# chalharu/rust-compression

Hardware: AMD Instinct MI355X
Metric: BZip2 level-9 encode MB/s (input bytes, HBM-resident in and out: the kernels' rate; value_end_to_end is host buffer to host buffer at the C ABI) (higher is better)
Workload: dtype u8/u32

## Files before the change

rust-compression_amd/csrc/k_bwt.hip:

```cpp
#include "bzgpu.h"
#include <algorithm>
#include <atomic>
#include <cstdio>
#include <cstdlib>
#include <vector>

namespace bzgpu {
constexpr u32 kGhSpan = 8;
constexpr u32 kSymSpan = 8;

enum { SRC_TEXT = 0, SRC_PAIRS = 1, SRC_MM = 2, SRC_WALK = 3, SRC_SURV = 4, SRC_LISTG = 5,
       SRC_TEXTK = 6, SRC_WALKK = 7, SRC_MMK = 8,
       SRC_MMC = 9,
       SRC_PERJ = 10,
       SRC_PACKED = 11,
       SRC_PERJK = 12,
       SRC_WALKA = 13 };
template <int SRC> struct src_is_list {
    static constexpr bool value = (SRC == SRC_PAIRS || SRC == SRC_SURV || SRC == SRC_LISTG || SRC == SRC_PERJ || SRC == SRC_PERJK || SRC == SRC_PACKED);
};

struct KeyInfo {
    u8 bits;
    u8 chars;
// ... 582 lines not shown
#pragma unroll
    for (u32 k = 0; k < 16; ++k) {
        const u32 i = k * kSortThreads + threadIdx.x;
        if (i < total) Vout[base + dst[k]] = s_buf[i];
    }
}

template <int B0, int B1, int B2>
__global__ __launch_bounds__(kSortThreads) void k_ghist_text(BwtArgs a, u32 *__restrict__ Kstore)
{
    constexpr u32 NB0 = 1u << B0, NB1 = 1u << B1, NB2 = 1u << B2;
    __shared__ u32 s_h0[2][NB0], s_h1[2][NB1], s_h2[2][NB2];
    u32 tile, lb;
    xcd_remap(gridDim.x, a.nb, tile, lb);
    if (lb == 0xFFFFFFFFu) return;
    const BlockDesc d = a.blocks[lb];
    const u32 n = d.n;
    const u32 start0 = tile * kGhSpan * kSortTile;
    if (start0 >= n) return;
    const u8 *text = a.rle + d.rle_off;
    const u8 *pt = a.ptext + (size_t)lb * kPtSlot;
    const KeyInfo ki = reinterpret_cast<const KeyInfo *>(a.keyinfo)[lb];
    if (B0 == 10 && B1 == 10 && B2 == 10 && !Kstore && counts_from_pack(ki)) return;
    for (u32 i = threadIdx.x; i < 2 * NB0; i += kSortThreads) (&s_h0[0][0])[i] = 0;
    for (u32 i = threadIdx.x; i < 2 * NB1; i += kSortThreads) (&s_h1[0][0])[i] = 0;
    for (u32 i = threadIdx.x; i < 2 * NB2; i += kSortThreads) (&s_h2[0][0])[i] = 0;
    __syncthreads();
    const u32 w = threadIdx.x >> 6, l = threadIdx.x & 63u;
    const size_t base = (size_t)lb * kSlot;
#pragma unroll 1
    for (u32 sp = 0; sp < kGhSpan; ++sp) {
        const u32 start = start0 + sp * kSortTile;
        if (start >= n) break;
        u32 key[16], val[16];
        const u32 ok = fetch_rows<SRC_TEXT>(a, lb, pt, n, 0, nullptr, nullptr, start + w * 1024u + l, n, ki, key, val);
#pragma unroll
        for (u32 r = 0; r < 16; ++r) {
            if ((ok >> r) & 1u) {
                atomicAdd(&s_h0[l & 1u][key[r] & (NB0 - 1)], 1u);
                atomicAdd(&s_h1[l & 1u][(key[r] >> B0) & (NB1 - 1)], 1u);
                atomicAdd(&s_h2[l & 1u][(key[r] >> (B0 + B1)) & (NB2 - 1)], 1u);
                if (Kstore) Kstore[base + start + w * 1024u + r * 64u + l] = key[r];
            }
        }
    }
    __syncthreads();
    u32 *out = a.gh_tiles + ((size_t)lb * kTilesPerBlock + tile) * 3 * kMaxBins;
    for (u32 i = threadIdx.x; i < NB0; i += kSortThreads) out[i] = s_h0[0][i] + s_h0[1][i];
    for (u32 i = threadIdx.x; i < NB1; i += kSortThreads) out[kMaxBins + i] = s_h1[0][i] + s_h1[1][i];
    for (u32 i = threadIdx.x; i < NB2; i += kSortThreads) out[2 * kMaxBins + i] = s_h2[0][i] + s_h2[1][i];
}

__global__ __launch_bounds__(kSortThreads) void k_ghist_scan(BwtArgs a, u32 ndig, u32 nbins0, u32 nbins1, u32 nbins2,
                                                             u32 ntiles_from_count, u32 span = 1u, u32 pack_counts = 0u)
{
    __shared__ u32 s_wsum[kSortThreads / 64];
    const u32 lb = blockIdx.x;
    const u32 n = a.blocks[lb].n;
    const u32 len = ntiles_from_count ? a.count[lb] : n;
    const u32 ntiles = ((len + kSortTile - 1) / kSortTile + span - 1u) / span;
    const u32 *gt = a.gh_tiles + (size_t)lb * kTilesPerBlock * 3 * kMaxBins;
    u32 total0 = 0;
    const bool one_set = pack_counts && counts_from_pack(reinterpret_cast<const KeyInfo *>(a.keyinfo)[lb]);
    if (one_set) ndig = 1;
    for (u32 dpos = 0; dpos < ndig; ++dpos) {
        const u32 nbins = dpos == 0 ? nbins0 : (dpos == 1 ? nbins1 : nbins2);
        const u32 per = (nbins + kSortThreads - 1) / kSortThreads;
        u32 tot[4] = {0, 0, 0, 0};
        u32 mine = 0;
        for (u32 q = 0; q < per; ++q) {
            const u32 bin = threadIdx.x * per + q;
            u32 sum = 0;
            if (bin < nbins)
                for (u32 t = 0; t < ntiles; ++t) sum += gt[(size_t)t * 3 * kMaxBins + dpos * kMaxBins + bin];
            tot[q] = sum;
            mine += sum;
        }
        const u32 inc = wave_incl_sum(mine);
        __syncthreads();
        if ((threadIdx.x & 63u) == 63u) s_wsum[threadIdx.x >> 6] = inc;
        __syncthreads();
        u32 carry = 0, total = 0;
        for (u32 k = 0; k < kSortThreads / 64; ++k) {
            if (k < (threadIdx.x >> 6)) carry += s_wsum[k];
            total += s_wsum[k];
        }
        u32 run = carry + inc - mine;
        for (u32 q = 0; q < per; ++q) {
            const u32 bin = threadIdx.x * per + q;
            if (bin < nbins) {
                a.gbase[((size_t)lb * 3 + dpos) * kMaxBins + bin] = run;
                if (one_set) {
                    a.gbase[((size_t)lb * 3 + 1) * kMaxBins + bin] = run;
                    a.gbase[((size_t)lb * 3 + 2) * kMaxBins + bin] = run;
                }
            }
            run += tot[q];
        }
        if (dpos == 0) total0 = total;
    }
    if (threadIdx.x == 0) a.count[lb] = total0;
}

#ifdef BZ_SCATTER_TIMING
#define SC_T(k) do { __syncthreads(); const u64 t_ = __builtin_readcyclecounter(); if (threadIdx.x == 0) atomicAdd(&a.loc_stats[32 + ((SRC == SRC_PAIRS || SRC == SRC_PACKED) ? 0 : 8) + (k)], (u32)((t_ - t_prev) >> 6)); t_prev = t_; } while (0)
#else
#define SC_T(k) do { } while (0)
#endif
template <int SRC, int BITS, bool WRITE_K = true, bool PACK_OUT = false, int ROWS = 16, int TILE = (int)kSortTile>
__global__ __launch_bounds__(TILE / ROWS) void k_radix_scatter_lb(BwtArgs a, u32 shift, u32 h,
                                                                    const u32 *__restrict__ Kin,
                                                                    const u32 *__restrict__ Vin,
                                                                    u32 *__restrict__ Kout, u32 *__restrict__ Vout,
                                                                    u32 dpos, u32 epoch,
                                                                    const u32 *__restrict__ gate)
{
    constexpr u32 NB = 1u << BITS;
    constexpr u32 kT = (u32)TILE / ROWS;
    static_assert((u32)TILE == kSortTile, "the look-back words are laid out for tiles of kSortTile elements");
    constexpr u32 kTileStride = kTilesPerBlock;
    u32 *const tstate = a.tile_state;
    constexpr u32 kRows = ROWS;
// ... 744 lines not shown
        if (h_next < n) atomicAdd(&a.active[round], (unsigned long long)s_nonfinal);
    }
    {
        const u32 b0 = threadIdx.x * 2u;
        const u32 c0 = s_bcnt[b0], c1 = s_bcnt[b0 + 1];
        const u32 mine = c0 + c1;
        const u32 inc = wave_incl_sum(mine);
        if (l == 63) s_wsum[w] = inc;
        u32 g0 = 0, g1 = 0;
        u32 *cur = a.bin_cursor + (size_t)lb * 1024u;
        if (c0) g0 = atomicAdd(&cur[b0], c0);
        if (c1) g1 = atomicAdd(&cur[b0 + 1], c1);
        __syncthreads();
        u32 carry = 0;
        for (u32 k = 0; k < w; ++k) carry += s_wsum[k];
        const u32 ex = carry + inc - mine;
        s_bpre[b0] = (u16)ex;
        s_bpre[b0 + 1] = (u16)(ex + c0);
        s_bcnt[b0] = (b0 << kRankBinShift) + g0;
        s_bcnt[b0 + 1] = ((b0 + 1u) << kRankBinShift) + g1;
    }
    __syncthreads();
#pragma unroll
    for (u32 r = 0; r < 16; ++r) {
        if (lrank[r] != 0xFFFFFFFFu) {
            const u32 bin = jv[r] >> kRankBinShift;
            const u32 pos = (u32)s_bpre[bin] + lrank[r];
            s_stage[pos] = word[r];
            s_binof[pos] = (u16)bin;
        }
    }
    __syncthreads();
    const u32 total = (cnt - start) < kSortTile ? (cnt - start) : kSortTile;
#pragma unroll
    for (u32 k = 0; k < 16; ++k) {
        const u32 i = k * kSortThreads + threadIdx.x;
        if (i < total) {
            const u32 bin = s_binof[i];
            W[base + s_bcnt[bin] + (i - (u32)s_bpre[bin])] = s_stage[i];
        }
    }
}

constexpr u32 kLbNone = 0xFFFFFu;
#ifdef BZ_REFINE_TIMING
#define RF_T(k) do { __syncthreads(); const u64 t_ = __builtin_readcyclecounter(); if (threadIdx.x == 0) atomicAdd(&a.loc_stats[16 + (INIT ? 8 : 0) + (k)], (u32)((t_ - t_prev) >> 4)); t_prev = t_; } while (0)
#else
#define RF_T(k) do { } while (0)
#endif
template <bool INIT, bool ABITS = false>
__global__ __launch_bounds__(kSortThreads, 4) void k_group_refine(BwtArgs a, u32 step, u32 next_step, u32 round,
                                                                const u32 *__restrict__ K,
                                                                const u32 *__restrict__ V, u32 *__restrict__ W,
                                                                u32 epoch)
{
    constexpr u32 NW = kSortThreads / 64;
    __shared__ int s_carry_old, s_carry_new;
    __shared__ int s_wold[NW], s_wnew[NW];
    __shared__ u32 s_nonfinal, s_ticket;
    __shared__ u32 s_stage[kSortTile];
    __shared__ u16 s_binof[kSortTile];
    __shared__ u16 s_bpre[1024];
    __shared__ u16 s_bdst[1024];
    __shared__ u32 s_wsum[NW];
    u32 (*s_gh)[1024] = reinterpret_cast<u32 (*)[1024]>(s_stage);
    u32 *s_bcnt = s_stage + 2048;
#ifdef BZ_REFINE_TIMING
    u64 t_prev = __builtin_readcyclecounter();
#endif
    const u32 xcd = (u32)__builtin_amdgcn_s_getreg(20 | (3 << 11)) & 7u;
    const u32 my_tiles = a.tiles * ((a.nb + 7u - xcd) / 8u);
    if (threadIdx.x == 0) s_ticket = atomicAdd(&a.tickets[(size_t)epoch * 8u + xcd], 1u);
    __syncthreads();
    const u32 slot = s_ticket;
    if (slot >= my_tiles) return;
    const u32 b8 = slot / a.tiles;
    const u32 tile = slot - b8 * a.tiles;
    const u32 lb = b8 * 8u + xcd;
    const BlockDesc d = a.blocks[lb];
    const u32 n = d.n;
    const u8 *__restrict__ text = a.rle + d.rle_off;
    const u32 cnt = a.count[lb];
    const u32 start = tile * kSortTile;
    if (start >= cnt) return;
    const KeyInfo ki = reinterpret_cast<const KeyInfo *>(a.keyinfo)[lb];
    const u32 hm = INIT ? (u32)ki.chars % n : (((u32)ki.chars * 2u) << step) % n;
    const u8 *pt = a.ptext + (size_t)lb * kPtSlot;
    const size_t base = (size_t)lb * kSlot;
    static_assert(INIT || !ABITS, "the boundary bitmap belongs to the init");
    if (INIT && !ABITS && a.pb_gate[lb] == 0u) K = a.KA;
    for (u32 i = threadIdx.x; i < 3072u; i += kSortThreads) s_stage[i] = 0;
    if (threadIdx.x == 0) s_nonfinal = 0;
    const u32 w = threadIdx.x >> 6, l = threadIdx.x & 63u;
    const u32 wbase = start + w * 1024u;
    const u32 first = wbase + l;

    RF_T(0);
    u32 gk[16], jv[16], s1[16], s2[16];
    u32 pg0 = 0, ps10 = 0, ps20 = 0;
    u32 ng0 = 0, ns10 = 0, ns20 = 0;
    const bool need_prev = (l == 0) && (first > 0) && (first < cnt);
    const bool need_next = (l == 63) && (wbase + 1024u < cnt);
    const u64 aword = ABITS ? newbits_lane_word(a.abits, base, wbase, cnt, l, false) : 0ull;
    {
#pragma unroll
        for (u32 r = 0; r < 16; ++r) {
            const u32 idx = first + r * 64u;
            const u32 c = idx < cnt ? idx : cnt - 1u;
            const u32 kk = ABITS ? 0u : ld_stream(K + base + c);
            const u32 vv = ld_stream(V + base + c);
            if (INIT) {
                jv[r] = vv;
                const u32 t = vv + hm;
                s2[r] = t >= n ? t - n : t;
                gk[r] = 0u;
                s1[r] = kk;
            } else {
                jv[r] = vv & 0xFFFFFu;
                gk[r] = kk & 0xFFFFFu;
                s1[r] = (kk >> 20) | ((vv >> 20) << 12);
                s2[r] = 0u;
            }
        }
        u32 pj = 0, nj = 0;
        if (need_prev) {
            const u32 kk = ABITS ? 0u : K[base + wbase - 1], vv = V[base + wbase - 1];
            pg0 = INIT ? 0u : (kk & 0xFFFFFu);
            ps10 = INIT ? kk : ((kk >> 20) | ((vv >> 20) << 12));
            const u32 t = vv + hm;
            pj = t >= n ? t - n : t;
        }
        if (need_next) {
            const u32 kk = ABITS ? 0u : K[base + wbase + 1024u], vv = V[base + wbase + 1024u];
            ng0 = INIT ? 0u : (kk & 0xFFFFFu);
            ns10 = INIT ? kk : ((kk >> 20) | ((vv >> 20) << 12));
            const u32 t = vv + hm;
            nj = t >= n ? t - n : t;
        }
        if (INIT) {
            pkey_rows(pt, s2, ki, s2);
            if (need_prev) ps20 = pkey(pt, pj, ki);
            if (need_next) ns20 = pkey(pt, nj, ki);
        }
    }
// ... 84 lines not shown
            }
            const u32 fi = etag | kLbIncl;
            const u32 io = lo >= 0 ? (u32)lo : (u32)co, in = ln >= 0 ? (u32)ln : (u32)cn;
            st_sc1_x4(mystate, make_uint4(fi | (io & kLbValMask), fi | (in & kLbValMask), fi, fi));
        }
        a.tile_last_new[lb * kTilesPerBlock + tile] = ln >= 0 ? ln : cn;
        a.tile_last_old[lb * kTilesPerBlock + tile] = lo >= 0 ? lo : co;
        s_carry_old = co;
        s_carry_new = cn;
    }
    __syncthreads();
    RF_T(3);
    int carry_old = INIT ? 0 : s_carry_old, carry_new = s_carry_new;
    for (u32 k = 0; k < w; ++k) {
        if (!INIT) carry_old = s_wold[k] > carry_old ? s_wold[k] : carry_old;
        carry_new = s_wnew[k] > carry_new ? s_wnew[k] : carry_new;
    }
    const u64 le_mask = (l == 63) ? ~0ull : ((2ull << l) - 1ull);
    u32 my_nonfinal = 0;
    u32 word[16], lrank[16];
#pragma unroll
    for (u32 r = 0; r < 16; ++r) {
        const u32 rowbase = wbase + r * 64u;
        const u32 idx = rowbase + l;
        lrank[r] = 0xFFFFFFFFu;
        word[r] = 0;
        bool nf = false;
        u32 nf_head = 0;
        if (idx < cnt) {
            int rs = 0;
            if (!INIT) {
                const u64 o = mo[r] & le_mask;
                rs = o ? (int)(rowbase + 63u - __clzll(o)) : carry_old;
            }
            const u64 q = mn[r] & le_mask;
            const int ss = q ? (int)(rowbase + 63u - __clzll(q)) : carry_new;
            const bool fin = (finbits >> r) & 1u;
            const u32 g = gk[r];
            const u32 j = jv[r];
            const u32 p = g + (idx - (u32)rs);
            const u32 head = g + ((u32)ss - (u32)rs);
            if (!INIT) st_stream(a.SA + base + p, j);
            if (fin) {
                a.L[base + p] = INIT ? (u8)lcol[r] : text[j ? j - 1u : n - 1u];
                if (j == 0) a.orig_ptr[lb] = p;
            }
            word[r] = (j & kRankBinMask) | (head << kRankBinShift) | (fin ? kFinalBit : 0u);
            lrank[r] = atomicAdd(&s_bcnt[j >> kRankBinShift], 1u);
            nf = !fin;
            nf_head = head;
        }
        {
            const u64 mnf = __ballot(nf);
            if (mnf) {
                my_nonfinal += (u32)__popcll(mnf);
                if (nf && (l == 0 || ((mn[r] >> l) & 1ull))) {
                    const u64 rest = (l == 63) ? 0ull : (mn[r] >> (l + 1u));
                    u32 len = rest ? (u32)__ffsll((long long)rest) : 64u - l;
                    len = len < cnt - idx ? len : cnt - idx;
                    atomicAdd(&s_gh[0][nf_head & 1023u], len);
                }
                const u32 lead = (u32)__ffsll((long long)mnf) - 1u;
                const u32 hi = (nf_head >> 10) & 1023u;
                const u32 hi0 = wave_lane(hi, lead);
                const u64 same = __ballot(nf && hi == hi0);
                if (same == mnf) {
                    if (l == lead) atomicAdd(&s_gh[1][hi0], (u32)__popcll(mnf));
                } else if (nf) {
                    atomicAdd(&s_gh[1][hi], 1u);
                }
            }
        }
        if (!INIT && mo[r]) carry_old = (int)(rowbase + 63u - __clzll(mo[r]));
        if (mn[r]) carry_new = (int)(rowbase + 63u - __clzll(mn[r]));
    }
    if (l == 0 && my_nonfinal) atomicAdd(&s_nonfinal, my_nonfinal);
    __syncthreads();
    RF_T(4);
    if (threadIdx.x == 0) a.tile_nf[lb * kTilesPerBlock + tile] = s_nonfinal;
    {
        u32 *out = a.gh_tiles + ((size_t)lb * kTilesPerBlock + tile) * 3 * kMaxBins;
        for (u32 i = threadIdx.x; i < 1024u; i += kSortThreads) {
            out[i] = s_gh[0][i];
            out[kMaxBins + i] = s_gh[1][i];
        }
    }
    if (threadIdx.x == 0 && s_nonfinal) {
        atomicMax(&a.maxnf[round], atomicAdd(&a.nonfinal[lb], s_nonfinal) + s_nonfinal);
        const u32 h_next = ((u32)ki.chars * 2u) << next_step;
        if (h_next < n) atomicAdd(&a.active[round], (unsigned long long)s_nonfinal);
    }
    {
        const u32 b0 = threadIdx.x * 2u;
        const u32 c0 = s_bcnt[b0], c1 = s_bcnt[b0 + 1];
        const u32 mine = c0 + c1;
        const u32 inc = wave_incl_sum(mine);
        if (l == 63) s_wsum[w] = inc;
        u32 g0 = 0, g1 = 0;
        u32 *cur = a.bin_cursor + (size_t)lb * 1024u;
        if (c0) g0 = atomicAdd(&cur[b0], c0);
        if (c1) g1 = atomicAdd(&cur[b0 + 1], c1);
        __syncthreads();
        u32 carry = 0;
        for (u32 k = 0; k < w; ++k) carry += s_wsum[k];
        const u32 ex = carry + inc - mine;
        s_bpre[b0] = (u16)ex;
        s_bpre[b0 + 1] = (u16)(ex + c0);
        s_bdst[b0] = (u16)g0;
        s_bdst[b0 + 1] = (u16)g1;
    }
    __syncthreads();
    RF_T(5);
#pragma unroll
    for (u32 r = 0; r < 16; ++r) {
        if (lrank[r] != 0xFFFFFFFFu) {
            const u32 bin = jv[r] >> kRankBinShift;
            const u32 pos = (u32)s_bpre[bin] + lrank[r];
            s_stage[pos] = word[r];
            s_binof[pos] = (u16)bin;
        }
    }
    __syncthreads();
    const u32 total = (cnt - start) < kSortTile ? (cnt - start) : kSortTile;
#pragma unroll
    for (u32 k = 0; k < 16; ++k) {
        const u32 i = k * kSortThreads + threadIdx.x;
        if (i < total) {
            const u32 bin = s_binof[i];
            W[base + (bin << kRankBinShift) + (u32)s_bdst[bin] + (i - (u32)s_bpre[bin])] = s_stage[i];
        }
    }
    RF_T(6);
}

__global__ __launch_bounds__(kSortThreads) void k_rank_place(BwtArgs a, const u32 *__restrict__ W)
{
    __shared__ u32 s_r[kSortThreads / 64][kRankBinSize];
    u32 tile, lb;
    xcd_remap(gridDim.x, a.nb, tile, lb);
    if (lb == 0xFFFFFFFFu) return;
    const u32 n = a.blocks[lb].n;
    const u32 w = threadIdx.x >> 6, l = threadIdx.x & 63u;
    const u32 bin = tile * (kSortThreads / 64) + w;
    const u32 j0 = bin << kRankBinShift;
    if (j0 >= n) return;
    const u32 c = a.bin_cursor[(size_t)lb * 1024u + bin];
    if (c == 0) return;
    const size_t base = (size_t)lb * kSlot + j0;
    const u32 span = (n - j0) < kRankBinSize ? (n - j0) : kRankBinSize;
    u32 *mine = s_r[w];
    if (c < 128u) {
        for (u32 i = l; i < c; i += 64u) {
            const u32 x = ld_stream(W + base + i);
            a.R[base + (x & kRankBinMask)] = ((x >> kRankBinShift) & 0xFFFFFu) | (x & kFinalBit);
        }
        return;
    }
    if (c == kRankBinSize) {
        typedef u32 u32x4 __attribute__((ext_vector_type(4)));
        const u32x4 *src = reinterpret_cast<const u32x4 *>(W + base);
        uint4 *dst = reinterpret_cast<uint4 *>(a.R + base);
        u32x4 q[kRankBinSize / 256];
#pragma unroll
        for (u32 k = 0; k < kRankBinSize / 256; ++k) q[k] = __builtin_nontemporal_load(src + k * 64u + l);
#pragma unroll
        for (u32 k = 0; k < kRankBinSize / 256; ++k) {
            const u32 x[4] = {q[k].x, q[k].y, q[k].z, q[k].w};
#pragma unroll
            for (u32 e = 0; e < 4; ++e) mine[x[e] & kRankBinMask] = ((x[e] >> kRankBinShift) & 0xFFFFFu) | (x[e] & kFinalBit);
        }
#pragma unroll
        for (u32 k = 0; k < kRankBinSize / 256; ++k) dst[k * 64u + l] = reinterpret_cast<const uint4 *>(mine)[k * 64u + l];
        return;
    }
    if (c < span)
        for (u32 i = l; i < span; i += 64u) mine[i] = a.R[base + i];
    for (u32 i = l; i < c; i += 64u) {
        const u32 x = ld_stream(W + base + i);
        mine[x & kRankBinMask] = ((x >> kRankBinShift) & 0xFFFFFu) | (x & kFinalBit);
    }
    for (u32 i = l; i < span; i += 64u) a.R[base + i] = mine[i];
}

__global__ __launch_bounds__(kSortThreads) void k_survivor_compact(BwtArgs a, const u32 *__restrict__ V,
                                                                    u32 *__restrict__ VS, u32 *__restrict__ midx = nullptr, u32 dense_only = 0)
{
    constexpr u32 NW = kSortThreads / 64;
    __shared__ u32 s_off, s_wsum[NW], s_total;
    u32 tile, lb;
    xcd_remap(gridDim.x, a.nb, tile, lb);
    if (lb == 0xFFFFFFFFu) return;
    const u32 cnt = a.count[lb];
    const u32 start = tile * kSortTile;
    const u32 ntiles = (cnt + kSortTile - 1) / kSortTile;
    if (tile == 0 && threadIdx.x == 0) {
        u32 tot = 0;
        for (u32 t = 0; t < ntiles; ++t) tot += a.tile_nf[lb * kTilesPerBlock + t];
        a.count2[lb] = tot;
    }
    if (start >= cnt) return;
    if (a.tile_nf[lb * kTilesPerBlock + tile] == 0) return;
    const size_t base = (size_t)lb * kSlot;
    if (threadIdx.x == 0) {
        u32 off = 0, tot = 0;
        for (u32 t = 0; t < tile; ++t) off += a.tile_nf[lb * kTilesPerBlock + t];
        if (midx && dense_only)
            for (u32 t = 0; t < ntiles; ++t) tot += a.tile_nf[lb * kTilesPerBlock + t];
        s_off = off;
        s_total = tot;
    }
    const u32 w = threadIdx.x >> 6, l = threadIdx.x & 63u;
    const u32 wbase = start + w * 1024u;
    u64 surv[16];
    u32 jv[16];
    u32 wcount = 0;
#pragma unroll
    for (u32 r = 0; r < 16; ++r) {
        const u32 idx = wbase + r * 64u + l;
        const u32 c = idx < cnt ? idx : cnt - 1u;
        jv[r] = ld_stream(V + base + c) & 0xFFFFFu;
    }
    u64 mn[17];
    {
        const u64 myword = newbits_lane_word(a.newbits, base, wbase, cnt, l, true);
#pragma unroll
        for (u32 r = 0; r < 17; ++r) mn[r] = wave_lane64(myword, r);
    }
    const u64 mn_prev = (midx && wbase >= 64u) ? a.newbits[(base + wbase - 64u) >> 6] : 0ull;
    u8 *gb8 = midx ? group_bytes(a, lb) : nullptr;
#pragma unroll
    for (u32 r = 0; r < 16; ++r) {
        const u32 idx = wbase + r * 64u + l;
        bool next_new;
        if (idx + 1 >= cnt) next_new = true;
        else if (l < 63) next_new = (mn[r] >> (l + 1)) & 1ull;
        else next_new = mn[r + 1] & 1ull;
        const bool is_new = (mn[r] >> l) & 1ull;
        const bool sv = (idx < cnt) && !(is_new && next_new);
        surv[r] = __ballot(sv);
        wcount += (u32)__popcll(surv[r]);
    }
    if (l == 0) s_wsum[w] = wcount;
    __syncthreads();
    u32 off = s_off;
    for (u32 k = 0; k < w; ++k) off += s_wsum[k];
    const u64 lt_mask = (l == 0) ? 0ull : (~0ull >> (64 - l));
    bool any_small = false;
    const bool sparse = midx && ((dense_only && (u64)s_total * 4u < (u64)a.blocks[lb].n) || a.blocks[lb].n < 64u);
#pragma unroll
    for (u32 r = 0; r < 16; ++r) {
        const u32 at = off + (u32)__popcll(surv[r] & lt_mask);
        if ((surv[r] >> l) & 1ull) VS[base + at] = jv[r];
        if (midx && ((surv[r] >> l) & 1ull)) {
            const u64 cur = mn[r], prv = r ? mn[r - 1] : mn_prev, nxw = mn[r + 1];
            const u64 lo = (l == 63u) ? cur : ((cur << (63u - l)) | (prv >> (l + 1u)));
            const u64 hi = (l == 63u) ? nxw : ((cur >> (l + 1u)) | (nxw << (63u - l)));
            const u32 back = lo ? (u32)__clzll(lo) : 64u, fwd = hi ? (u32)__builtin_ctzll(hi) + 1u : 65u;
            const u32 size = back + fwd;
            const bool small = size >= 2u && size <= kLinkMax && !sparse;
            gb8[at] = small ? (u8)(back | (size << 4)) : (u8)0;
            if (small) {
                midx[base + jv[r]] = at | (back << 20) | (size << 24);
                any_small = true;
            }
        }
        off += (u32)__popcll(surv[r]);
    }
    if (any_small) a.ptext[base + kSlot - 2u] = 1;
}

__global__ void k_copy_counts(u32 *__restrict__ dst, const u32 *__restrict__ src, u32 nb)
{
    const u32 i = blockIdx.x * blockDim.x + threadIdx.x;
    if (i < nb) dst[i] = src[i];
}

__global__ __launch_bounds__(kSortThreads) void k_periodic_stats(BwtArgs a)
{
    u32 tile, lb;
    xcd_remap(gridDim.x, a.nb, tile, lb);
    if (lb == 0xFFFFFFFFu) return;
    if (a.nonfinal[lb] == 0) return;
    const u32 n = a.blocks[lb].n;
    const size_t base = (size_t)lb * kSlot;
    u32 c = 0, mj = 0xFFFFFFFFu;
    for (u32 j = tile * kSortTile + threadIdx.x; j < n && j < (tile + 1) * kSortTile; j += kSortThreads) {
        if (a.R[base + j] == 0u) {
            ++c;
            mj = j < mj ? j : mj;
        }
    }
    c = wave_sum(c);
#pragma unroll
    for (u32 dd = 32; dd >= 1; dd >>= 1) {
        const u32 o = __shfl_xor(mj, dd, 64);
        mj = o < mj ? o : mj;
    }
    if ((threadIdx.x & 63u) == 0 && c) {
        atomicAdd(&a.per_k[lb], c);
        atomicMin(&a.per_shift[lb], mj);
    }
}

__global__ __launch_bounds__(kSortThreads) void k_periodic_place(BwtArgs a)
{
    u32 tile, lb;
    xcd_remap(gridDim.x, a.nb, tile, lb);
    if (lb == 0xFFFFFFFFu) return;
    if (a.nonfinal[lb] == 0) return;
    const BlockDesc d = a.blocks[lb];
    const u32 n = d.n;
    const u8 *__restrict__ text = a.rle + d.rle_off;
    const size_t base = (size_t)lb * kSlot;
    const u32 k = a.per_k[lb], shift = a.per_shift[lb];
    if (k == 0) return;
    const u32 p = n / k;
    for (u32 j = tile * kSortTile + threadIdx.x; j < n && j < (tile + 1) * kSortTile; j += kSortThreads) {
        const u32 r = a.R[base + j];
        if (r & kFinalBit) continue;
        const u32 i0 = j % p, t = j / p;
        const u32 pos = (i0 >= shift) ? (k - 1u - t) : (t == 0 ? 0u : k - t);
// ... 1115 lines not shown
    static const bool want_refine = !(getenv("BZ_FUSED_REFINE") && atoi(getenv("BZ_FUSED_REFINE")) == 0);
    static const bool want_abits = !(getenv("BZ_INIT_ABITS") && atoi(getenv("BZ_INIT_ABITS")) == 0);
    const bool abits = fused && want_refine && want_abits && a.abits != nullptr;
    if (fused) {
        const bool ok = wide_keys ? init_sort_fused<11, 11, 10>(st, a, total_n, prof, abits) : init_sort_fused<10, 10, 10>(st, a, total_n, prof, abits);
        if (!ok) {
            fprintf(stderr, "bz2_mi355x: fused radix passes disabled (tile tickets / look-back check failed)\n");
            a.fused_state[0] = 1;
            a.fused_state[1] += 1;
            fused = false;
            a.fused = 0;
            (void)hipMemsetAsync(a.sort_err, 0, 4, st);
        }
    }
    if (!fused) {
        (void)hipMemsetAsync(a.pb_gate, 1, a.nb * sizeof(u32), st);
        if (wide_keys) init_sort<11, 11, 10>(st, a, total_n, prof);
        else init_sort<10, 10, 10>(st, a, total_n, prof);
    }
    const bool refine = fused && want_refine;
    int p;
    (void)hipMemsetAsync(a.bin_cursor, 0, (size_t)a.nb * 1024 * sizeof(u32), st);
    if (refine) {
        const u32 e = next_epoch(st, a);
        p = prof ? prof->begin(st, KID_GROUP_REFINE, abits ? total_n * 10 + total_n / 8 : total_n * 14) : -1;
        if (abits) hipLaunchKernelGGL((k_group_refine<true, true>), grid, dim3(kSortThreads), 0, st, a, 0u, 0u, 0u, (const u32 *)nullptr, a.SA, a.KA, e);
        else hipLaunchKernelGGL((k_group_refine<true>), grid, dim3(kSortThreads), 0, st, a, 0u, 0u, 0u, a.KB, a.SA, a.KA, e);
        if (prof) prof->end(st, p);
    } else {
        p = prof ? prof->begin(st, KID_GROUP_FLAGS, total_n * 9) : -1;
        hipLaunchKernelGGL((k_group_flags<true>), grid, dim3(kSortThreads), 0, st, a, 0u, a.KB, a.SA);
        if (prof) prof->end(st, p);
        p = prof ? prof->begin(st, KID_GROUP_APPLY, total_n * 13) : -1;
        hipLaunchKernelGGL((k_group_apply<true>), grid, dim3(kSortThreads), 0, st, a, 0u, 0u, a.KB, a.SA, a.KA);
        if (prof) prof->end(st, p);
    }
    p = prof ? prof->begin(st, KID_RANK_PLACE, total_n * 8) : -1;
    hipLaunchKernelGGL(k_rank_place, grid, dim3(kSortThreads), 0, st, a, a.KA);
    if (prof) prof->end(st, p);

    u32 *cK = a.KB, *cV = a.VB;
    u32 *fK = a.KA, *fV = a.VA;
    const u32 *lastV = a.SA;
    u32 step = 0;
    int rounds = 0;
    u32 slot = 0;
    bool period_done = false;
    bool last_doubled = false, links_pay = true;
    u64 link_m = 0;
    if (!(a.gh_tiles && a.per_aux)) a.per_links = 0;
    const u32 links_on = a.per_links;
    bool surv_local_ok = true;
    u32 list_tiles = a.tiles;
    while (true) {
        {
            const MailSeg sg[2] = {{h_active, a.active + slot, sizeof(unsigned long long)}, {h_active + 1, a.maxnf + slot, sizeof(u32)}};
            if (mail_fetch(st, sg, 2) != 0) return -1;
        }
        const u64 m = *h_active;
        const u32 list_tiles_prev = list_tiles;
        const u32 mx = *reinterpret_cast<const u32 *>(h_active + 1);
        {
            list_tiles = (mx + kSortTile - 1) / kSortTile + 1u;
            if (list_tiles > kTilesPerBlock) list_tiles = kTilesPerBlock;
        }
        const dim3 grid_list(list_tiles, xcd_grid_y(a.nb)), grid_prev(list_tiles_prev, xcd_grid_y(a.nb));
        if (sorted_elems) *sorted_elems += m;
        if (round_active && slot < 64) round_active[slot] += m;
        if (m == 0 || step > 24 || ((u64)(2u * min_chars) << step) >= max_n) break;
        ++slot;
        ++rounds;
        bool carried = false;
        u32 trace_worst = 0;
        static const bool bwt_trace = getenv("BZ_BWT_TRACE") != nullptr;
        if (bwt_trace) {
            std::vector<u32> nf(a.nb);
            (void)hipMemcpyAsync(nf.data(), a.nonfinal, a.nb * 4, hipMemcpyDeviceToHost, st);
            (void)hipStreamSynchronize(st);
            trace_worst = (u32)(std::max_element(nf.begin(), nf.end()) - nf.begin());
        }
        (void)hipMemsetAsync(a.nonfinal, 0, a.nb * sizeof(u32), st);
        static const int want_period = [] {
            const char *e = getenv("BZ_PERIOD_ROUND");
            return !e ? 1 : (e[0] == 'b' ? 2 : (atoi(e) != 0 ? 1 : 0));
        }();
        const bool deep = want_period == 2 ? (rounds >= 3 && m * 4 >= total_n * 3)
                                           : ((rounds >= 2 && ((u64)mx * 4 >= (u64)max_n * 3 || m * 4 >= total_n * 3)) ||
                                              (rounds == 1 && m * 64 >= total_n * 63));
        const bool per_round = want_period != 0 && !period_done && deep;
        if (link_m) {
            if ((link_m - m) * 4 < link_m) links_pay = false;
            link_m = 0;
        }
        const bool link_round = !per_round && links_on && period_done && last_doubled && links_pay && m * 256 >= total_n;
        constexpr u64 surv_num = 1, surv_den = 4;
        if (bwt_trace)
            fprintf(stderr, "bz2_mi355x: sort round %d (h = %llu): %llu of %llu rotations unordered, at most %u in one block (block %u; of %u)%s\n",
                    rounds, (unsigned long long)(2u * min_chars) << step, (unsigned long long)m, (unsigned long long)total_n, mx,
                    trace_worst, max_n, per_round ? ": period round" : (link_round ? ": link round" : (m * surv_den < total_n * surv_num ? ": survivor form" : ": walk form")));
        u8 *impure = a.ptext;
        last_doubled = !(per_round || link_round);
        if (per_round || link_round) {
            if (per_round) period_done = true;
            else link_m = m;
            (void)hipMemsetAsync(impure, 0, (size_t)a.nb * kSlot, st);
            const bool links = links_on != 0 && !(per_round && rounds == 1);
// ... 8 lines not shown
                (void)hipMemsetAsync(a.lin_p, 0, (size_t)a.nb * kPerK * 4, st);
                hipLaunchKernelGGL(k_link_compact, grid_list, dim3(kSortThreads), 0, st, a, fV, cK, cV);
            } else {
            hipLaunchKernelGGL(k_period_find, dim3(a.nb), dim3(kSortThreads), 0, st, a, 3u);
            hipLaunchKernelGGL(k_period_bits, grid, dim3(kSortThreads), 0, st, a);
            hipLaunchKernelGGL(k_period_next, dim3(a.nb, per_kmax(a)), dim3(kSortThreads), 0, st, a);
            bool one_pass = false, wide = false;
            {
                std::vector<u32> lp((size_t)a.nb * kPerK), ls((size_t)a.nb * kPerK);
                {
                    const MailSeg sg[2] = {{lp.data(), a.lin_p, lp.size() * 4}, {ls.data(), a.lin_sig, ls.size() * 4}};
                    if (mail_fetch(st, sg, 2) != 0) return -1;
                }
                one_pass = true;
                u32 small = 0, smallest = 0xFFFFFFFFu;
                const u64 depth_max = 16ull << step;
                for (size_t i = 0; i < lp.size(); ++i) {
                    if (lp[i] != 0u && lp[i] < 1024u && ls[i] >= 200u) {
                        one_pass = false;
                        small += 1;
                        smallest = lp[i] < smallest ? lp[i] : smallest;
                    }
                    if (lp[i] != 0u && lp[i] <= depth_max) wide = true;
                }
                if (wide) one_pass = false;
                if (bwt_trace) fprintf(stderr, "  period round: %s (%u distances below 1024 that a fifth of their block agrees at, the smallest %u)\n", wide ? "three passes over thirty-bit keys" : (one_pass ? "one pass over the keys" : "two passes over the keys"), small, small ? smallest : 0u);
            }
            a.per_keyshift = one_pass ? 10u : 0u;
            a.per_wide = wide ? 1u : 0u;
            if (one_pass) {
                radix_pass<SRC_PERJ, 10>(st, a, 0, step, nullptr, fV, cK, cV, m, prof, fK, list_tiles);
                radix_pass<SRC_LISTG, 10>(st, a, 0, step, nullptr, cV, fK, cK, m, prof, fV, list_tiles);
                radix_pass<SRC_PAIRS, 10>(st, a, 10, step, fK, cK, cV, fV, m, prof, nullptr, list_tiles);
                u32 *rk = cV, *rv = fV, *ok = fK, *ov = cK;
                cK = rk; cV = rv; fK = ok; fV = ov;
            } else if (wide) {
                radix_pass<SRC_PERJ, 10>(st, a, 0, step, nullptr, fV, cK, cV, m, prof, fK, list_tiles);
                radix_pass<SRC_PAIRS, 10>(st, a, 10, step, cK, cV, fK, fV, m, prof, nullptr, list_tiles);
                radix_pass<SRC_PAIRS, 10>(st, a, 20, step, fK, fV, cK, cV, m, prof, nullptr, list_tiles);
                radix_pass<SRC_LISTG, 10>(st, a, 0, step, nullptr, cV, fK, fV, m, prof, cK, list_tiles);
                radix_pass<SRC_PAIRS, 10>(st, a, 10, step, fK, fV, cK, cV, m, prof, nullptr, list_tiles);
            } else {
                radix_pass<SRC_PERJ, 10>(st, a, 0, step, nullptr, fV, cK, cV, m, prof, fK, list_tiles);
                radix_pass<SRC_PAIRS, 10>(st, a, 10, step, cK, cV, fK, fV, m, prof, nullptr, list_tiles);
                radix_pass<SRC_LISTG, 10>(st, a, 0, step, nullptr, fV, cK, cV, m, prof, fK, list_tiles);
                radix_pass<SRC_PAIRS, 10>(st, a, 10, step, cK, cV, fK, fV, m, prof, nullptr, list_tiles);
                u32 *t = cK; cK = fK; fK = t;
                t = cV; cV = fV; fV = t;
            }
            a.per_keyshift = 0;
            hipLaunchKernelGGL(k_period_mark, grid_list, dim3(kSortThreads), 0, st, a, step, cK, cV, impure);
            }
        } else if (m * surv_den < total_n * surv_num) {
            hipLaunchKernelGGL(k_survivor_compact, grid_prev, dim3(kSortThreads), 0, st, a, lastV, fV);
            hipLaunchKernelGGL(k_copy_counts, dim3((a.nb + 255) / 256), dim3(256), 0, st, a.count, a.count2, a.nb);
            bool local_done = false;
            if (surv_local_ok && m * 8 < total_n) {
                u32 fails = 0;
                (void)hipMemsetAsync(a.loc_stats + LOC_STAT_SURV_FAIL, 0, 4, st);
                hipLaunchKernelGGL(k_surv_local, grid_list, dim3(kLocThreads), 0, st, a, step, fV, cK, cV);
                {
                    const MailSeg sg = {&fails, a.loc_stats + LOC_STAT_SURV_FAIL, 4};
                    if (mail_fetch(st, &sg, 1) != 0) return -1;
                }
                local_done = fails == 0;
                if (!local_done) surv_local_ok = false;
                if (bwt_trace) fprintf(stderr, "  survivor round inside LDS: %s\n", local_done ? "done" : "a segment did not fit or failed its check: the global passes");
            }
            if (!local_done) {
            radix_pass<SRC_SURV, 10>(st, a, 0, step, nullptr, fV, cK, cV, m, prof, fK, list_tiles);
            radix_pass<SRC_PAIRS, 10>(st, a, 10, step, cK, cV, fK, fV, m, prof, nullptr, list_tiles);
            radix_pass<SRC_LISTG, 10>(st, a, 0, step, nullptr, fV, cK, cV, m, prof, fK, list_tiles);
            radix_pass<SRC_PAIRS, 10>(st, a, 10, step, cK, cV, fK, fV, m, prof, nullptr, list_tiles);
            u32 *t = cK; cK = fK; fK = t;
            t = cV; cV = fV; fV = t;
            }
        } else {
            if (fused) {
                hipLaunchKernelGGL(k_ghist_scan, dim3(a.nb), dim3(kSortThreads), 0, st, a, 2u, 1024u, 1024u, 0u, 1u);
                carried = refine && rounds == 1;
                if (carried) fused_pass<SRC_MMC, 10>(st, a, 0, step, nullptr, nullptr, fK, fV, 0, total_n, prof, m);
                else fused_pass<SRC_MM, 10>(st, a, 0, step, nullptr, nullptr, fK, fV, 0, total_n, prof, m);
                fused_pass<SRC_PAIRS, 10>(st, a, 10, step, fK, fV, cK, cV, 1, m, prof);
            } else {
                radix_pass<SRC_MM, 10>(st, a, 0, step, nullptr, nullptr, fK, fV, total_n, prof, cK);
                radix_pass<SRC_PAIRS, 10>(st, a, 10, step, fK, fV, cK, cV, m, prof);
            }
        }
        (void)hipMemsetAsync(a.bin_cursor, 0, (size_t)a.nb * 1024 * sizeof(u32), st);
        if (per_round || link_round) {
            p = prof ? prof->begin(st, KID_GROUP_FLAGS, m * 13) : -1;
            hipLaunchKernelGGL((k_group_flags<false>), grid_list, dim3(kSortThreads), 0, st, a, step, cK, cV, impure);
            a.per_wide = 0;
            a.per_links = links_on;
            if (prof) prof->end(st, p);
            p = prof ? prof->begin(st, KID_GROUP_APPLY, m * 17) : -1;
            hipLaunchKernelGGL((k_group_apply<false>), grid_list, dim3(kSortThreads), 0, st, a, step, slot, cK, cV, fK);
            if (prof) prof->end(st, p);
        } else if (carried) {
            const u32 e = next_epoch(st, a);
            p = prof ? prof->begin(st, KID_GROUP_REFINE, m * 18) : -1;
            hipLaunchKernelGGL((k_group_refine<false>), grid, dim3(kSortThreads), 0, st, a, step, step + 1, slot, cK, cV, fK, e);
            if (prof) prof->end(st, p);
        } else {
            p = prof ? prof->begin(st, KID_GROUP_FLAGS, m * 13) : -1;
            hipLaunchKernelGGL((k_group_flags<false>), grid_list, dim3(kSortThreads), 0, st, a, step, cK, cV);
            if (prof) prof->end(st, p);
            p = prof ? prof->begin(st, KID_GROUP_APPLY, m * 17) : -1;
            hipLaunchKernelGGL((k_group_apply<false>), grid_list, dim3(kSortThreads), 0, st, a, step + 1, slot, cK, cV, fK);
            if (prof) prof->end(st, p);
        }
        p = prof ? prof->begin(st, KID_RANK_PLACE, m * 8) : -1;
        hipLaunchKernelGGL(k_rank_place, grid, dim3(kSortThreads), 0, st, a, fK);
        if (prof) prof->end(st, p);
        if (per_round && bwt_trace) {
            std::vector<u32> lp((size_t)a.nb * kPerK), ls((size_t)a.nb * kPerK), nf(a.nb), cn(a.nb);
            (void)hipMemcpyAsync(lp.data(), a.lin_p, (size_t)a.nb * kPerK * 4, hipMemcpyDeviceToHost, st);
            (void)hipMemcpyAsync(ls.data(), a.lin_sig, (size_t)a.nb * kPerK * 4, hipMemcpyDeviceToHost, st);
            (void)hipMemcpyAsync(nf.data(), a.nonfinal, a.nb * 4, hipMemcpyDeviceToHost, st);
            (void)hipMemcpyAsync(cn.data(), a.count, a.nb * 4, hipMemcpyDeviceToHost, st);
            (void)hipStreamSynchronize(st);
            for (u32 b = 0; b < a.nb; ++b)
                if (lp[(size_t)b * kPerK] || nf[b] * 2u > max_n) {
                    fprintf(stderr, "  block %u: distances (agreement in permille of the block)", b);
                    for (u32 i = 0; i < kPerK && lp[(size_t)b * kPerK + i]; ++i) fprintf(stderr, " %u (%u)", lp[(size_t)b * kPerK + i], ls[(size_t)b * kPerK + i]);
                    fprintf(stderr, "; list %u, %u rotations left unordered\n", cn[b], nf[b]);
                }
        }
        lastV = cV;
        if (!per_round && !link_round) ++step;
    }
    if (fused) {
        u32 gave_up = 0;
        std::vector<u32> tk;
        const u32 epoch_last = *a.epoch;
        if (epoch_last >= epoch_first)
            tk.resize((size_t)(epoch_last - epoch_first + 1u) * 8u);
        {
            const MailSeg sg[2] = {{&gave_up, a.sort_err, 4}, {tk.data(), a.tickets + (size_t)epoch_first * 8u, tk.size() * 4}};
            if (mail_fetch(st, sg, tk.empty() ? 1 : 2) != 0) return -1;
        }
        static const bool late_fail_test = getenv("BZ_ONESWEEP_LATEFAILTEST") != nullptr;
        bool bad = gave_up != 0 || late_fail_test;
        for (size_t i = 0; i < tk.size(); ++i)
            if (tk[i] != a.tiles * (xcd_grid_y(a.nb) / 8u)) bad = true;
        if (bad) {
            (void)hipMemsetAsync(a.sort_err, 0, 4, st);
            return -2;
        }
    }
#if defined(BZ_SCATTER_TIMING) || defined(BZ_REFINE_TIMING)
    {
        (void)hipStreamSynchronize(st);
#ifdef BZ_SCATTER_TIMING
        {
            u32 rt[16] = {};
            (void)hipMemcpy(rt, a.loc_stats + 32, sizeof(rt), hipMemcpyDeviceToHost);
            fprintf(stderr, "  k_radix_scatter_lb cycles/64 per phase (set-up, fetch+rank, scans, look-back, stage K, store K, stage V, store V): "
                            "streamed sources %u %u %u %u %u %u %u %u; gathering sources %u %u %u %u %u %u %u %u\n", rt[0], rt[1], rt[2], rt[3],
                    rt[4], rt[5], rt[6], rt[7], rt[8], rt[9], rt[10], rt[11], rt[12], rt[13], rt[14], rt[15]);
            (void)hipMemset(a.loc_stats + 32, 0, sizeof(rt));
            u32 lk[4] = {};
            (void)hipMemcpy(lk, a.loc_stats + 48, sizeof(lk), hipMemcpyDeviceToHost);
            fprintf(stderr, "  look-back of thread 0's digits: %u tiles, %u hops (%.2f per tile, most %u), %u repeated loads (%.2f per tile)\n", lk[2], lk[0],
                    lk[2] ? (double)lk[0] / lk[2] : 0.0, lk[3], lk[1], lk[2] ? (double)lk[1] / lk[2] : 0.0);
            (void)hipMemset(a.loc_stats + 48, 0, sizeof(lk));
        }
#endif
#ifdef BZ_REFINE_TIMING
        {
            u32 rt[16] = {};
            (void)hipMemcpy(rt, a.loc_stats + 16, sizeof(rt), hipMemcpyDeviceToHost);
            fprintf(stderr, "  k_group_refine cycles/16 per phase (set-up, list+keys, flags, look-back, apply, counts, out): first refinement "
                            "%u %u %u %u %u %u %u; walk round %u %u %u %u %u %u %u\n", rt[8], rt[9], rt[10], rt[11], rt[12], rt[13], rt[14],
                    rt[0], rt[1], rt[2], rt[3], rt[4], rt[5], rt[6]);
            (void)hipMemset(a.loc_stats + 16, 0, sizeof(rt));
        }
#endif
    }
#endif
    (void)hipMemsetAsync(a.per_k, 0, a.nb * sizeof(u32), st);
    (void)hipMemsetAsync(a.per_shift, 0xFF, a.nb * sizeof(u32), st);
// ... 29 lines not shown
```

Measured before the change: 15290.

## Emit survivors and packed histograms from refine to skip compaction and histogram work

In the non-init refine kernel, each tile now writes its non-final rotation indices straight to a scratch buffer at ballot-computed offsets. A new gather kernel then builds the survivor list by copying per-tile prefixes, replacing the full survivor-compact pass after carried rounds. The init refine packs its two 1024-bin digit histograms as 16-bit pairs to halve the histogram traffic, and the scan kernel gains a narrow mode to read them. After carried rounds a separate walk-counts kernel recomputes the histograms from R, which adds a kernel and an extra scratch write in return for skipping the compaction scan.

```diff
diff --git a/rust-compression_amd/csrc/k_bwt.hip b/rust-compression_amd/csrc/k_bwt.hip
--- a/rust-compression_amd/csrc/k_bwt.hip
+++ b/rust-compression_amd/csrc/k_bwt.hip
@@ -658,7 +658,8 @@
 }
 
 __global__ __launch_bounds__(kSortThreads) void k_ghist_scan(BwtArgs a, u32 ndig, u32 nbins0, u32 nbins1, u32 nbins2,
-                                                             u32 ntiles_from_count, u32 span = 1u, u32 pack_counts = 0u)
+                                                             u32 ntiles_from_count, u32 span = 1u, u32 pack_counts = 0u,
+                                                             u32 narrow = 0u)
 {
     __shared__ u32 s_wsum[kSortThreads / 64];
     const u32 lb = blockIdx.x;
@@ -674,6 +675,15 @@
         const u32 per = (nbins + kSortThreads - 1) / kSortThreads;
         u32 tot[4] = {0, 0, 0, 0};
         u32 mine = 0;
+        if (narrow && nbins == 2u * kSortThreads) {
+            const u32 *g = gt + dpos * (kMaxBins / 2u) + threadIdx.x;
+            for (u32 t = 0; t < ntiles; ++t) {
+                const u32 v = g[(size_t)t * 3 * kMaxBins];
+                tot[0] += v & 0xFFFFu;
+                tot[1] += v >> 16;
+            }
+            mine = tot[0] + tot[1];
+        } else
         for (u32 q = 0; q < per; ++q) {
             const u32 bin = threadIdx.x * per + q;
             u32 sum = 0;
@@ -1524,12 +1534,13 @@
 __global__ __launch_bounds__(kSortThreads, 4) void k_group_refine(BwtArgs a, u32 step, u32 next_step, u32 round,
                                                                 const u32 *__restrict__ K,
                                                                 const u32 *__restrict__ V, u32 *__restrict__ W,
-                                                                u32 epoch)
+                                                                u32 epoch, u32 *__restrict__ S = nullptr)
 {
     constexpr u32 NW = kSortThreads / 64;
     __shared__ int s_carry_old, s_carry_new;
     __shared__ int s_wold[NW], s_wnew[NW];
     __shared__ u32 s_nonfinal, s_ticket;
+    __shared__ u32 s_wnf[NW];
     __shared__ u32 s_stage[kSortTile];
     __shared__ u16 s_binof[kSortTile];
     __shared__ u16 s_bpre[1024];
@@ -1561,7 +1572,7 @@
     const size_t base = (size_t)lb * kSlot;
     static_assert(INIT || !ABITS, "the boundary bitmap belongs to the init");
     if (INIT && !ABITS && a.pb_gate[lb] == 0u) K = a.KA;
-    for (u32 i = threadIdx.x; i < 3072u; i += kSortThreads) s_stage[i] = 0;
+    for (u32 i = (INIT ? 0u : 2048u) + threadIdx.x; i < 3072u; i += kSortThreads) s_stage[i] = 0;
     if (threadIdx.x == 0) s_nonfinal = 0;
     const u32 w = threadIdx.x >> 6, l = threadIdx.x & 63u;
     const u32 wbase = start + w * 1024u;
@@ -1752,8 +1763,8 @@
         }
         {
             const u64 mnf = __ballot(nf);
-            if (mnf) {
-                my_nonfinal += (u32)__popcll(mnf);
+            my_nonfinal += (u32)__popcll(mnf);
+            if (INIT && mnf) {
                 if (nf && (l == 0 || ((mn[r] >> l) & 1ull))) {
                     const u64 rest = (l == 63) ? 0ull : (mn[r] >> (l + 1u));
                     u32 len = rest ? (u32)__ffsll((long long)rest) : 64u - l;
@@ -1775,14 +1786,27 @@
         if (mn[r]) carry_new = (int)(rowbase + 63u - __clzll(mn[r]));
     }
     if (l == 0 && my_nonfinal) atomicAdd(&s_nonfinal, my_nonfinal);
+    if (!INIT && l == 0) s_wnf[w] = my_nonfinal;
     __syncthreads();
     RF_T(4);
     if (threadIdx.x == 0) a.tile_nf[lb * kTilesPerBlock + tile] = s_nonfinal;
-    {
+    if (!INIT && s_nonfinal) {
+        u32 at = start;
+        for (u32 k = 0; k < w; ++k) at += s_wnf[k];
+        const u64 lt_mask = (l == 0) ? 0ull : (~0ull >> (64 - l));
+#pragma unroll
+        for (u32 r = 0; r < 16; ++r) {
+            const bool nf = lrank[r] != 0xFFFFFFFFu && !(word[r] & kFinalBit);
+            const u64 mnf = __ballot(nf);
+            if (nf) S[base + at + (u32)__popcll(mnf & lt_mask)] = jv[r];
+            at += (u32)__popcll(mnf);
+        }
+    }
+    if (INIT) {
         u32 *out = a.gh_tiles + ((size_t)lb * kTilesPerBlock + tile) * 3 * kMaxBins;
-        for (u32 i = threadIdx.x; i < 1024u; i += kSortThreads) {
-            out[i] = s_gh[0][i];
-            out[kMaxBins + i] = s_gh[1][i];
+        for (u32 i = threadIdx.x; i < 512u; i += kSortThreads) {
+            out[i] = s_gh[0][2u * i] | (s_gh[0][2u * i + 1u] << 16);
+            out[kMaxBins / 2u + i] = s_gh[1][2u * i] | (s_gh[1][2u * i + 1u] << 16);
         }
     }
     if (threadIdx.x == 0 && s_nonfinal) {
@@ -1882,6 +1906,45 @@
     for (u32 i = l; i < span; i += 64u) a.R[base + i] = mine[i];
 }
 
+__global__ __launch_bounds__(kSortThreads) void k_walk_counts(BwtArgs a)
+{
+    __shared__ u32 s_h0[2][1024], s_h1[2][1024];
+    u32 tile, lb;
+    xcd_remap(gridDim.x, a.nb, tile, lb);
+    if (lb == 0xFFFFFFFFu) return;
+    const u32 n = a.blocks[lb].n;
+    const u32 ltiles = (a.count[lb] + kSortTile - 1) / kSortTile;
+    if (tile >= ltiles) return;
+    for (u32 i = threadIdx.x; i < 2048u; i += kSortThreads) {
+        (&s_h0[0][0])[i] = 0;
+        (&s_h1[0][0])[i] = 0;
+    }
+    __syncthreads();
+    const u32 *R = a.R + (size_t)lb * kSlot;
+    const u32 c = threadIdx.x & 1u;
+    for (u32 start = tile * kSortTile; start < n; start += ltiles * kSortTile) {
+        u32 x[16];
+#pragma unroll
+        for (u32 r = 0; r < 16; ++r) {
+            const u32 j = start + r * kSortThreads + threadIdx.x;
+            x[r] = j < n ? ld_stream(R + j) : kFinalBit;
+        }
+#pragma unroll
+        for (u32 r = 0; r < 16; ++r) {
+            if (!(x[r] & kFinalBit)) {
+                atomicAdd(&s_h0[c][x[r] & 1023u], 1u);
+                atomicAdd(&s_h1[c][(x[r] >> 10) & 1023u], 1u);
+            }
+        }
+    }
+    __syncthreads();
+    u32 *out = a.gh_tiles + ((size_t)lb * kTilesPerBlock + tile) * 3 * kMaxBins;
+    for (u32 i = threadIdx.x; i < 1024u; i += kSortThreads) {
+        out[i] = s_h0[0][i] + s_h0[1][i];
+        out[kMaxBins + i] = s_h1[0][i] + s_h1[1][i];
+    }
+}
+
 __global__ __launch_bounds__(kSortThreads) void k_survivor_compact(BwtArgs a, const u32 *__restrict__ V,
                                                                     u32 *__restrict__ VS, u32 *__restrict__ midx = nullptr, u32 dense_only = 0)
 {
@@ -1967,6 +2030,34 @@
         off += (u32)__popcll(surv[r]);
     }
     if (any_small) a.ptext[base + kSlot - 2u] = 1;
+}
+
+__global__ __launch_bounds__(kSortThreads) void k_survivor_gather(BwtArgs a, const u32 *__restrict__ S, u32 *__restrict__ VS)
+{
+    __shared__ u32 s_off;
+    u32 tile, lb;
+    xcd_remap(gridDim.x, a.nb, tile, lb);
+    if (lb == 0xFFFFFFFFu) return;
+    const u32 cnt = a.count[lb];
+    const u32 start = tile * kSortTile;
+    const u32 ntiles = (cnt + kSortTile - 1) / kSortTile;
+    const u32 *nfs = a.tile_nf + lb * kTilesPerBlock;
+    if (threadIdx.x < 64u) {
+        const u32 upto = tile == 0 ? ntiles : (tile < ntiles ? tile : 0u);
+        u32 v = 0;
+        for (u32 t = threadIdx.x; t < upto; t += 64u) v += nfs[t];
+        v = wave_sum(v);
+        if (threadIdx.x == 0) {
+            if (tile == 0) a.count2[lb] = v;
+            s_off = tile == 0 ? 0u : v;
+        }
+    }
+    if (start >= cnt) return;
+    const u32 nf = nfs[tile];
+    __syncthreads();
+    const size_t base = (size_t)lb * kSlot;
+    const u32 off = s_off;
+    for (u32 i = threadIdx.x; i < nf; i += kSortThreads) VS[base + off + i] = ld_stream(S + base + start + i);
 }
 
 __global__ void k_copy_counts(u32 *__restrict__ dst, const u32 *__restrict__ src, u32 nb)
@@ -3188,6 +3279,7 @@
     const u32 links_on = a.per_links;
     bool surv_local_ok = true;
     u32 list_tiles = a.tiles;
+    bool prev_carried = false;
     while (true) {
         {
             const MailSeg sg[2] = {{h_active, a.active + slot, sizeof(unsigned long long)}, {h_active + 1, a.maxnf + slot, sizeof(u32)}};
@@ -3302,7 +3394,12 @@
             hipLaunchKernelGGL(k_period_mark, grid_list, dim3(kSortThreads), 0, st, a, step, cK, cV, impure);
             }
         } else if (m * surv_den < total_n * surv_num) {
-            hipLaunchKernelGGL(k_survivor_compact, grid_prev, dim3(kSortThreads), 0, st, a, lastV, fV);
+            if (prev_carried) {
+                hipLaunchKernelGGL(k_survivor_gather, grid_prev, dim3(kSortThreads), 0, st, a, fV, cV);
+                std::swap(cV, fV);
+            } else {
+                hipLaunchKernelGGL(k_survivor_compact, grid_prev, dim3(kSortThreads), 0, st, a, lastV, fV);
+            }
             hipLaunchKernelGGL(k_copy_counts, dim3((a.nb + 255) / 256), dim3(256), 0, st, a.count, a.count2, a.nb);
             bool local_done = false;
             if (surv_local_ok && m * 8 < total_n) {
@@ -3327,7 +3424,9 @@
             }
         } else {
             if (fused) {
-                hipLaunchKernelGGL(k_ghist_scan, dim3(a.nb), dim3(kSortThreads), 0, st, a, 2u, 1024u, 1024u, 0u, 1u);
+                if (prev_carried) hipLaunchKernelGGL(k_walk_counts, grid_prev, dim3(kSortThreads), 0, st, a);
+                hipLaunchKernelGGL(k_ghist_scan, dim3(a.nb), dim3(kSortThreads), 0, st, a, 2u, 1024u, 1024u, 0u, 1u, 1u, 0u,
+                                   (refine && rounds == 1) ? 1u : 0u);
                 carried = refine && rounds == 1;
                 if (carried) fused_pass<SRC_MMC, 10>(st, a, 0, step, nullptr, nullptr, fK, fV, 0, total_n, prof, m);
                 else fused_pass<SRC_MM, 10>(st, a, 0, step, nullptr, nullptr, fK, fV, 0, total_n, prof, m);
@@ -3350,7 +3449,7 @@
         } else if (carried) {
             const u32 e = next_epoch(st, a);
             p = prof ? prof->begin(st, KID_GROUP_REFINE, m * 18) : -1;
-            hipLaunchKernelGGL((k_group_refine<false>), grid, dim3(kSortThreads), 0, st, a, step, step + 1, slot, cK, cV, fK, e);
+            hipLaunchKernelGGL((k_group_refine<false>), grid, dim3(kSortThreads), 0, st, a, step, step + 1, slot, cK, cV, fK, e, fV);
             if (prof) prof->end(st, p);
         } else {
             p = prof ? prof->begin(st, KID_GROUP_FLAGS, m * 13) : -1;
@@ -3378,6 +3477,7 @@
                 }
         }
         lastV = cV;
+        prev_carried = carried;
         if (!per_round && !link_round) ++step;
     }
     if (fused) {
```

Result: faster. 15470, median of 6 (+1.2%).
